# nianticlabs/implicit-depth

Hardware: AMD Instinct MI355X
Metric: frames/sec (BDModel.forward hot path, 512x384, 64 planes, 8-frame tuple = 1 current + 7 source views; third-party backbones excluded) (higher is better)
Workload: dtype f32

## Files before the change

implicit-depth_amd/csrc/conv.hip:

```cpp
#include <algorithm>
#include "conv_args.h"
#include "../../include/idh_ops.h"

using namespace idh_conv;

int idh_stem_op(const idh_op &op, hipStream_t st, bool launch);

namespace {

__device__ float g_zero_page[kZeroFloats];

thread_local bool t_dry_run = false;
thread_local int t_launches = 0;
#undef IDH_CHECK_LAUNCH
#define IDH_CHECK_LAUNCH()                                              \
    do {                                                                \
        if (!t_dry_run && hipGetLastError() != hipSuccess) return IDH_ELAUNCH; \
    } while (0)
#define IDH_LAUNCH(...)                         \
    do {                                        \
        if (t_dry_run) ++t_launches;            \
        else hipLaunchKernelGGL(__VA_ARGS__);   \
    } while (0)

// ... 1034 lines not shown
                ss[u][0] = fmaf(d0, d0, ss[u][0]); ss[u][1] = fmaf(d1, d1, ss[u][1]); ss[u][2] = fmaf(d2, d2, ss[u][2]); ss[u][3] = fmaf(d3, d3, ss[u][3]);
            }
        }
    }
#pragma unroll
    for (int u = 0; u < SUB; ++u) {
        float *mine = red + ((size_t)(prow + u * pstep) * cq + q) * 8;
#pragma unroll
        for (int e = 0; e < 4; ++e) { mine[e] = s[u][e]; mine[4 + e] = ss[u][e]; }
    }
    __syncthreads();
    for (int t = threadIdx.x; t < 8 * cq; t += blockDim.x) {
        const int qq = t >> 3, e = t & 7;
        float a = 0.f;
        for (int r = 0; r < rows; ++r) a += red[(r * cq + qq) * 8 + e];
        part[((size_t)(n * nchunks + chunk) * 2 + (e >> 2)) * C + 4 * qq + (e & 3)] = a;
    }
}

__global__ __launch_bounds__(256) void instnorm_finalize_k(const float *__restrict__ part, const float *__restrict__ in, int cs, int C, int HW,
                                                           int nchunks, float *__restrict__ stats) {
    const int n = blockIdx.x;
    for (int c = threadIdx.x; c < C; c += 256) {
        float s = 0.f, ss = 0.f;
        for (int k = 0; k < nchunks; ++k) {
            const float *o = part + ((size_t)(n * nchunks + k) * 2) * C + c;
            s += o[0];
            ss += o[C];
        }
        const float ms = s / (float)HW;
        const float var = fmaxf(ss / (float)HW - ms * ms, 0.f);
        stats[(size_t)n * 2 * C + c] = in[(size_t)n * HW * cs + c] + ms;
        stats[(size_t)n * 2 * C + C + c] = 1.0f / sqrtf(var + 1e-5f);
    }
}

__global__ __launch_bounds__(256) void instnorm_apply_k(const float *__restrict__ in, int cs, float *__restrict__ out, int out_cs,
                                                        int C, int HW, long long total, const float *__restrict__ stats, int act,
                                                        float slope) {
    const int cq = C >> 2;
    for (long long t = blockIdx.x * 256ll + threadIdx.x; t < total; t += gridDim.x * 256ll) {
        const int q = (int)(t % cq);
        const long long np = t / cq;
        const int n = (int)(np / HW);
        const float4 mean = *reinterpret_cast<const float4 *>(stats + (size_t)n * 2 * C + 4 * q);
        const float4 rstd = *reinterpret_cast<const float4 *>(stats + (size_t)n * 2 * C + C + 4 * q);
        const float4 v = *reinterpret_cast<const float4 *>(in + (size_t)np * cs + 4 * q);
        float r[4] = {(v.x - mean.x) * rstd.x, (v.y - mean.y) * rstd.y, (v.z - mean.z) * rstd.z, (v.w - mean.w) * rstd.w};
        for (int e = 0; e < 4; ++e) r[e] = act_apply(r[e], act, slope);
        *reinterpret_cast<float4 *>(out + (size_t)np * out_cs + 4 * q) = make_float4(r[0], r[1], r[2], r[3]);
    }
}

enum { LV_LDS4 = 0, LV_LDS2 = 1, LV_MFMA14 = 2, LV_UP2 = 3 };
struct LevelArgs {
    int n;
    unsigned start[kMaxGroup + 1];
    int kind[kMaxGroup];
    LdsConvArgs op[kMaxGroup];
};

template <bool WIDE>
__global__ __launch_bounds__(256) void level_k(const LevelArgs g) {
    __shared__ f32x4 sA[lds_a_slots(1)];
    __shared__ f32x4 sB[lds_b_slots(WIDE ? 4 : 2)];
    int idx = 0;
// ... 241 lines not shown
        g.start[i] = cursor;
        g.kind[i] = kinds[i];
        g.op[i] = pcs[i].la;
        if (kinds[i] == LV_MFMA14) g.op[i].c = pcs[i].a;
        cursor += pcs[i].blocks;
    }
    g.start[n] = cursor;
    bool wide = false;
    for (int i = 0; i < n; ++i) wide = wide || kinds[i] == LV_LDS4;
    if (wide) IDH_LAUNCH(level_k<true>, dim3(cursor), dim3(256), 0, st, g);
    else IDH_LAUNCH(level_k<false>, dim3(cursor), dim3(256), 0, st, g);
    IDH_CHECK_LAUNCH();
    return launch_reduces(pcs, n, st);
}

int level_kind(const PreparedConv &pc) {
    if (pc.up || pc.norm || pc.s2) return -1;
    if (pc.lds_rows == 4 && pc.nj == 4) return LV_LDS4;
    if (pc.lds_rows == 4 && pc.nj == 2) return LV_LDS2;
    if (pc.lds_rows == 0 && pc.tm == 1 && pc.tn == 4) return LV_MFMA14;
    return -1;
}

int check_upsample(const idh_op &op) {
    const idh_conv_src &s = op.src[0];
    if (!s.in || !op.out || (s.Cin & 3) || (s.cs & 3) || (op.out_cs & 3) || op.N <= 0 || s.H <= 0 || s.W <= 0 || s.Cin <= 0) return IDH_EINVAL;
    if ((long long)op.N * s.H * s.W * (s.Cin >> 2) >= (1ll << 31)) return IDH_EUNSUPPORTED;
    return IDH_OK;
}

constexpr unsigned kLevelMaxBlocks = 512;
constexpr unsigned kLevelUpsampleBlocks = 512;
constexpr long long kLevelUpsampleNatural = 4096;

}

extern "C" size_t idh_sizeof_op(void) { return sizeof(idh_op); }

extern "C" size_t idh_packed_weight_floats(int Cout, int Cin, int ks) {
    if (Cout <= 0 || Cin <= 0 || ks <= 0) return 0;
    return (size_t)ks * ks * ceil16(Cin) * ceil16(Cout);
}

extern "C" int idh_pack_conv_weight(const float *w, float *dst, int Cout, int Cin, int ks, void *stream) {
    if (!w || !dst || Cout <= 0 || Cin <= 0 || (ks != 1 && ks != 3)) return IDH_EINVAL;
    const long long total = (long long)idh_packed_weight_floats(Cout, Cin, ks);
    int grid = idh_cdiv(total, 256);
    if (grid > 4096) grid = 4096;
    hipLaunchKernelGGL(pack_weight_k, dim3(grid), dim3(256), 0, idh_stream(stream), w, dst, Cout, Cin, ks, ceil16(Cin),
                       ceil16(Cout));
    IDH_CHECK_LAUNCH();
    return IDH_OK;
}

extern "C" int idh_run_ops(const idh_op *ops, int n, void *stream) {
    if (n < 0 || (n > 0 && !ops)) return IDH_EINVAL;
    hipStream_t st = idh_stream(stream);
    for (int i = 0; i < n; ++i) {
        const idh_op &op = ops[i];
        const idh_conv_src &s = op.src[0];
        switch (op.kind) {
            case IDH_OP_CONV:
            case IDH_OP_UPSAMPLE2: {
                PreparedConv pcs[kMaxGroup];
                int kinds[kMaxGroup];
                int run = 0;
// ... 122 lines not shown
                IDH_CHECK_LAUNCH();
                break;
            }
            case IDH_OP_NHWC_TO_NCHW: {
                if (!s.in || !op.out || op.N <= 0 || op.N > 65535 || s.H <= 0 || s.W <= 0 || s.Cin <= 0 || s.cs < s.Cin) return IDH_EINVAL;
                const int HW = s.H * s.W;
                IDH_LAUNCH(export_nchw_k, dim3(idh_cdiv(HW, 64), idh_cdiv(s.Cin, 32), op.N), dim3(256), 0, st, s.in,
                                   op.out, s.Cin, HW, s.cs);
                IDH_CHECK_LAUNCH();
                break;
            }
            case IDH_OP_POINTWISE_HEAD: {
                if (!s.in || !s.w || !op.out || (s.Cin & 3) || (s.cs & 3) || op.N <= 0 || s.H <= 0 || s.W <= 0 || s.Cin <= 0 || s.cs < s.Cin)
                    return IDH_EINVAL;
                const long long M = (long long)op.N * s.H * s.W;
                int grid = idh_cdiv(M, 256);
                if (grid > 8192) grid = 8192;
                IDH_LAUNCH(pointwise_head_k, dim3(grid), dim3(256), 0, st, s.in, s.w, op.bias, op.out, op.ws, M, s.Cin,
                                   s.cs);
                IDH_CHECK_LAUNCH();
                break;
            }
            case IDH_OP_POINTWISE_NCHW: {
                if (!s.in || !s.w || !op.out || op.N <= 0 || s.H <= 0 || s.W <= 0 || (op.out_cs & 3) || ((uintptr_t)op.out & 15) ||
                    (op.bias && ((uintptr_t)op.bias & 15)))
                    return IDH_EINVAL;
                if (s.Cin != kPwCin || op.Cout != kPwCout || op.out_cs < kPwCout || (long long)s.H * s.W * kPwCin * 4 >= (1ll << 31))
                    return IDH_EUNSUPPORTED;
                PwNchwArgs pa{};
                pa.in = s.in; pa.w = s.w; pa.bias = op.bias; pa.out = op.out;
                pa.HW = s.H * s.W; pa.out_cs = op.out_cs;
                pa.tiles_per_img = idh_cdiv(pa.HW, kPwTile);
                pa.tiles = (long long)op.N * pa.tiles_per_img;
                const int grid = (int)std::min<long long>(pa.tiles, 256 * 4 * 4);
                IDH_LAUNCH(pointwise_nchw_k, dim3(grid), dim3(256), 0, st, pa);
                IDH_CHECK_LAUNCH();
                break;
            }
            case IDH_OP_POINTWISE_UP: {
                const idh_conv_src &lo = op.src[1];
                if (!s.in || !s.w || !lo.in || !op.out || op.N <= 0 || s.H <= 0 || s.W <= 0 || (s.H & 1) || (s.W & 1) || (s.cs & 3) || (lo.cs & 3) || (op.out_cs & 3) ||
                    s.cs < s.Cin || lo.cs < op.Cout || op.out_cs < op.Cout || ((uintptr_t)s.in & 15) || ((uintptr_t)lo.in & 15) || ((uintptr_t)op.out & 15) ||
                    ((uintptr_t)s.w & 15) || (op.bias && ((uintptr_t)op.bias & 15)) || lo.H != s.H / 2 || lo.W != s.W / 2)
                    return IDH_EINVAL;
                if (s.Cin != op.Cout || (s.Cin != 64 && s.Cin != 128) || (long long)s.H * s.W >= (1ll << 31)) return IDH_EUNSUPPORTED;
                PwUpArgs pa{};
                pa.in = s.in; pa.w = s.w; pa.bias = op.bias; pa.low = lo.in; pa.out = op.out;
                pa.H = s.H; pa.W = s.W; pa.in_cs = s.cs; pa.low_cs = lo.cs; pa.out_cs = op.out_cs;
                pa.tiles_per_img = idh_cdiv(s.H * s.W, kPwTile);
                pa.tiles = (long long)op.N * pa.tiles_per_img;
                const int grid = (int)std::min<long long>(pa.tiles, 256 * 8);
                if (s.Cin == 64) IDH_LAUNCH((pointwise_up_k<4, 4>), dim3(grid), dim3(256), 16 * 64 * sizeof(f32x4), st, pa);
                else IDH_LAUNCH((pointwise_up_k<8, 8>), dim3(grid), dim3(256), 32 * 128 * sizeof(f32x4), st, pa);
                IDH_CHECK_LAUNCH();
                break;
            }
            case IDH_OP_STEM: {
                const int rc = idh_stem_op(op, st, !t_dry_run);
                if (rc != IDH_OK) return rc;
                if (t_dry_run) ++t_launches;
                break;
            }
            case IDH_OP_COPY: {
                if (!s.in || !op.out || (s.Cin & 3) || (s.cs & 3) || (op.out_cs & 3) || op.N <= 0 || s.H <= 0 || s.W <= 0 || s.Cin <= 0 ||
                    s.cs < s.Cin || op.out_cs < s.Cin)
                    return IDH_EINVAL;
                const long long npix = (long long)op.N * s.H * s.W;
                int grid = idh_cdiv(npix * (s.Cin >> 2), 256);
                if (grid > 8192) grid = 8192;
                IDH_LAUNCH(copy_nhwc_k, dim3(grid), dim3(256), 0, st, s.in, op.out, npix, s.Cin, s.cs, op.out_cs);
                IDH_CHECK_LAUNCH();
                break;
            }
            case IDH_OP_INSTNORM: {
                const int C = s.Cin, HW = s.H * s.W;
                if (!s.in || !op.ws || C <= 0 || (C & 3) || 256 % (C >> 2) || (s.cs & 3) || (op.out && (op.out_cs & 3)) ||
                    op.N <= 0 || op.N > 65535 || s.H <= 0 || s.W <= 0)
                    return IDH_EINVAL;
                const int nchunks = idh_cdiv(HW, kInChunk);
                const int sthreads = ((long long)nchunks * op.N < 512 && C >= 64) ? 1024 : 256;
                if (C >= 64 && sthreads == 256)
                    IDH_LAUNCH(instnorm_stats_k<4>, dim3(nchunks, op.N), dim3(256), 1024 * 8 * sizeof(float), st, s.in, s.cs, C, HW, nchunks, op.ws);
                else
                    IDH_LAUNCH(instnorm_stats_k<1>, dim3(nchunks, op.N), dim3(sthreads), sthreads * 8 * sizeof(float), st, s.in, s.cs, C, HW,
                                       nchunks, op.ws);
                IDH_CHECK_LAUNCH();
                float *stats = op.ws + (size_t)op.N * nchunks * 2 * C;
                IDH_LAUNCH(instnorm_finalize_k, dim3(op.N), dim3(256), 0, st, op.ws, s.in, s.cs, C, HW, nchunks, stats);
                IDH_CHECK_LAUNCH();
                if (!op.out) break;
                const long long total = (long long)op.N * HW * (C >> 2);
                int gx = idh_cdiv(total, 256 * 4);
                if (gx > 16384) gx = 16384;
                IDH_LAUNCH(instnorm_apply_k, dim3(gx), dim3(256), 0, st, s.in, s.cs, op.out, op.out_cs, C, HW, total, stats, op.act,
                                   op.slope);
                IDH_CHECK_LAUNCH();
                break;
            }
            default:
                return IDH_EINVAL;
        }
    }
    return IDH_OK;
}

extern "C" int idh_conv_variant(const idh_op *op, int32_t out[8]) {
    if (!op || !out || op->kind != IDH_OP_CONV) return IDH_EINVAL;
    PreparedConv pc{};
    const int rc = prep_conv(*op, pc);
    if (rc != IDH_OK) return rc;
    const bool lds = pc.lds_rows == 8 || pc.lds_rows == 4;
    out[0] = pc.lds_rows;
    out[1] = lds ? pc.nj : 0;
    out[2] = lds ? 0 : pc.tm;
// ... 16 lines not shown
```

implicit-depth_amd/csrc/networks.hip:

```cpp
#include <algorithm>
#include <cstring>
#include <map>
#include <tuple>
#include <vector>

#include "idh_common.h"
#include "net_plan.h"
#include "../../include/idh_net.h"
#include "../../include/idh_ops.h"

namespace {

constexpr long long kReuseMinBytes = 64ll << 20;
constexpr bool kFuseHeadNorm = true;
constexpr bool kFuseHeadImport = true;

inline int ceil16(int v) { return (v + 15) & ~15; }
inline int cdiv(int a, int b) { return (a + b - 1) / b; }
inline size_t align64(size_t v) { return (v + 63) & ~(size_t)63; }

__global__ __launch_bounds__(256) void bias_sum_k(const float *__restrict__ a, const float *__restrict__ b, float *__restrict__ out, int n) {
    const int i = blockIdx.x * 256 + threadIdx.x;
    if (i < n) out[i] = (a ? a[i] : 0.f) + (b ? b[i] : 0.f);
}

enum Mode { MODE_SIZES, MODE_PACK, MODE_RUN };

struct Buf {
    float *base;
    int N, H, W, cs;
    bool internal;
    bool zero_fill;
    size_t floats;
};

struct View {
    int buf = -1, c0 = 0, C = 0;
};

struct Region {
    uint64_t buf, c0, c1;
};

struct Meta {
    std::vector<Region> reads, writes;
};

struct Src {
// ... 194 lines not shown
    }
    void export_nchw(const View &x, float *dst) {
        if (err) return;
        idh_op op;
        std::memset(&op, 0, sizeof op);
        op.kind = IDH_OP_NHWC_TO_NCHW; op.N = N(x);
        idh_conv_src &s = op.src[0];
        s.in = ptr(x); s.cs = cs(x); s.H = H(x); s.W = W(x); s.Cin = x.C;
        op.out = mode_ == MODE_RUN ? dst : reinterpret_cast<float *>(uintptr_t(4) << 32);
        ops.push_back(op);
        meta.push_back(Meta{{region(x)}, {}});
    }
    void head(const View &x, const idh_conv_params &cv, float *out, float *out_exp) {
        if (err) return;
        if (cv.cout != 1 || cv.ks != 1 || cv.cin != x.C) { err = IDH_EINVAL; return; }
        float *w = blob_alloc(cv.cin), *b = blob_alloc(1);
        if (mode_ == MODE_PACK) {
            if (!cv.weight || !cv.bias) { err = IDH_EINVAL; return; }
            if (hipMemcpyAsync(w, cv.weight, sizeof(float) * cv.cin, hipMemcpyDeviceToDevice, st_) != hipSuccess ||
                hipMemcpyAsync(b, cv.bias, sizeof(float), hipMemcpyDeviceToDevice, st_) != hipSuccess) err = IDH_ELAUNCH;
        }
        idh_op op;
        std::memset(&op, 0, sizeof op);
        op.kind = IDH_OP_POINTWISE_HEAD; op.N = N(x);
        idh_conv_src &s = op.src[0];
        s.in = ptr(x); s.w = w; s.cs = cs(x); s.H = H(x); s.W = W(x); s.Cin = x.C;
        op.bias = b;
        op.out = mode_ == MODE_RUN ? out : reinterpret_cast<float *>(uintptr_t(5) << 32);
        op.ws = mode_ == MODE_RUN ? out_exp : nullptr;
        ops.push_back(op);
        meta.push_back(Meta{{region(x)}, {}});
    }

    Norm instance_norm(const View &x, const View *out, int act, float slope) {
        Norm nm;
        if (err) return nm;
        if (x.C % 4 || 256 % (x.C / 4)) { err = IDH_EINVAL; return nm; }
        const int nchunks = cdiv(H(x) * W(x), 1024);
        float *w = ws_alloc((size_t)N(x) * (nchunks + 1) * 2 * x.C);
        idh_op op;
        std::memset(&op, 0, sizeof op);
        op.kind = IDH_OP_INSTNORM; op.N = N(x);
        idh_conv_src &s = op.src[0];
        s.in = ptr(x); s.cs = cs(x); s.H = H(x); s.W = W(x); s.Cin = x.C;
        op.act = act; op.slope = slope;
        if (out) { op.out = ptr(*out); op.out_cs = cs(*out); }
        op.ws = w;
        ops.push_back(op);
        Meta m{{region(x)}, {}};
        if (out) {
            m.writes.push_back(region(*out));
        } else {
            Buf b{};
            b.base = w + (size_t)N(x) * nchunks * 2 * x.C; b.N = N(x); b.H = 1; b.W = 1; b.cs = 1; b.internal = false;
            bufs.push_back(b);
            nm.stats = b.base; nm.buf = (int)bufs.size() - 1;
            m.writes.push_back(Region{(uint64_t)nm.buf, 0, 1});
        }
        meta.push_back(m);
        return nm;
    }
    static bool pointwise_nchw_eligible(const idh_conv_params &c) { return c.ks == 1 && c.stride == 1 && c.cin == 64 && c.cout == 128; }
    void pointwise_nchw(const float *src, int n, int C, int H_, int W_, const idh_conv_params &cv, const View &out) {
        if (err) return;
        if (n != N(out) || H_ != H(out) || W_ != W(out) || C != cv.cin || out.C != cv.cout || !pointwise_nchw_eligible(cv)) { err = IDH_EINVAL; return; }
        idh_op op;
        std::memset(&op, 0, sizeof op);
        op.kind = IDH_OP_POINTWISE_NCHW; op.N = n;
        idh_conv_src &s = op.src[0];
        s.in = mode_ == MODE_RUN ? src : reinterpret_cast<const float *>(uintptr_t(6) << 32);
        s.w = packed(cv, IDH_W_DIRECT); s.H = H_; s.W = W_; s.Cin = C; s.ks = 1; s.stride = 1;
        op.bias = bias_of(cv, nullptr);
        op.out = ptr(out); op.out_cs = cs(out); op.Ho = H_; op.Wo = W_; op.Cout = cv.cout;
        ops.push_back(op);
        meta.push_back(Meta{{}, {region(out)}});
    }

    void stem(const float *images, int n, int h, int w, const float *blob, const View &out) {
        if (err) return;
        idh_op op;
// ... 285 lines not shown
        if (i && (feats[i].H * 2 != feats[i - 1].H || feats[i].W * 2 != feats[i - 1].W)) return IDH_EINVAL;
        prev.push_back(input_view(p, feats[i], N));
    }
    return unetpp_body(p, blocks, heads, N, prev, fouts, log_depth, depth, nullptr, scales, true);
}

uint64_t layout_hash(const std::vector<idh_op> &ops) {
    uint64_t h = 1469598103934665603ull;
    auto mix = [&](long long v) {
        for (int i = 0; i < 8; ++i) { h ^= (uint64_t)((v >> (8 * i)) & 0xff); h *= 1099511628211ull; }
    };
    for (const idh_op &op : ops) {
        mix(op.kind); mix(op.N); mix(op.Ho); mix(op.Wo); mix(op.Cout); mix(op.tile_m); mix(op.tile_n); mix(op.split_k); mix(op.act); mix(op.group);
        for (const idh_conv_src &s : op.src) { mix(s.Cin); mix(s.H); mix(s.W); mix(s.cs); mix(s.ks); mix(s.stride); mix(s.pad_mode); mix(s.norm != nullptr); }
    }
    return h;
}

}

int idh_internal::conv_stage(int mode, ConvStage *s, float *ws, size_t ws_cap, float *blob, hipStream_t st, int (*before_ops)(void *), void *ctx) {
    const Mode m = mode == STAGE_SIZES ? MODE_SIZES : mode == STAGE_PACK ? MODE_PACK : MODE_RUN;
    if (!s || !s->enc || s->n_enc != 4 || !s->dec || s->N <= 0 || s->H <= 0 || s->W <= 0 || s->D <= 0) return IDH_EINVAL;
    Plan p(m, ws, ws_cap, blob, st);
    s->match = nullptr;
    s->n_head_ops = 0;
    if (s->head_mode) {
        if (!s->head || s->K <= 0 || (s->head_mode != 1 && s->head_mode != 2)) return IDH_EINVAL;
        const idh_conv_params &c1 = s->head[0], &c2 = s->head[1];
        const int M = s->N * (s->K + 1), H = s->H, W = s->W;
        if (c1.ks != 1 || c1.stride != 1 || c2.ks != 3 || c2.stride != 1 || c2.cin != c1.cout) return IDH_EINVAL;
        if (m == MODE_RUN && (!s->layer1 || ((uintptr_t)s->layer1 & 15))) return IDH_EINVAL;
        const View h = p.buffer(M, H, W, c1.cout);
        if (s->head_mode == 1 && kFuseHeadImport && Plan::pointwise_nchw_eligible(c1)) {
            p.pointwise_nchw(s->layer1, M, c1.cin, H, W, c1, h);
        } else {
            View x;
            if (s->head_mode == 1) {
                x = p.buffer(M, H, W, c1.cin);
                p.import_nchw(s->layer1, M, c1.cin, H, W, x);
            } else {
                const idh_tensor t{const_cast<float *>(s->layer1), IDH_LAYOUT_NHWC, c1.cin, H, W, c1.cin};
                if (!tensor_ok(&t, m == MODE_RUN)) return IDH_EINVAL;
                x = p.external(t, M);
            }
            p.conv(x, c1, h, IDH_ACT_NONE, 0.2f, nullptr, nullptr, nullptr);
        }
        const View y = p.buffer(M, H, W, c2.cout);
        idh_conv_choice hc;
        if (p.select({{h, &c2}}, y, IDH_ACT_NONE, 0.2f, nullptr, IDH_PAD_REPLICATE, false, false, &hc) != IDH_OK) return IDH_EINVAL;
        if (kFuseHeadNorm && h.C % 16 == 0 && hc.lds_subtiles == 1 && (hc.families & IDH_FAMILY_LDS)) {
            const Norm nm = p.instance_norm(h, nullptr, IDH_ACT_NONE, 0.2f);
            Norm on = nm;
            on.act = IDH_ACT_LRELU; on.slope = 0.2f;
            p.conv(h, c2, y, IDH_ACT_NONE, 0.2f, nullptr, nullptr, nullptr, IDH_PAD_REPLICATE, &on);
        } else {
            const View hn = p.buffer(M, H, W, c1.cout);
            p.instance_norm(h, &hn, IDH_ACT_LRELU, 0.2f);
            p.conv(hn, c2, y, IDH_ACT_NONE, 0.2f, nullptr, nullptr, nullptr, IDH_PAD_REPLICATE);
        }
        const View mo = p.buffer(M, H, W, c2.cout);
        p.instance_norm(y, &mo, IDH_ACT_NONE, 0.2f);
        if (p.err) return p.err;
        if (p.cs(mo) != mo.C) return IDH_EUNSUPPORTED;
        s->match = p.ptr(mo);
        s->n_head_ops = (int)p.ops.size();
    }
    const View cv_in = p.buffer(s->N, s->H, s->W, s->D);
    for (int i = 0; i < 5; ++i)
        if (s->img[i].layout != IDH_LAYOUT_NCHW || !tensor_ok(&s->img[i], m == MODE_RUN)) return IDH_EINVAL;
    const View v0 = input_view(p, s->img[0], s->N);
    std::vector<View> levels{v0};
    int rc = cvencoder_body(p, s->enc, s->n_enc, s->N, cv_in, &s->img[1], nullptr, &levels);
    if (rc != IDH_OK) return rc;
    for (int i = 1; i < 5; ++i)
        if (p.H(levels[i]) * 2 != p.H(levels[i - 1]) || p.W(levels[i]) * 2 != p.W(levels[i - 1])) return IDH_EINVAL;
    View f0;
    rc = unetpp_body(p, s->dec, s->heads, s->N, levels, nullptr, s->log_depth, s->depth, &f0, s->scales);
    if (rc != IDH_OK) return rc;
    s->cv_in = p.ptr(cv_in);
    s->cv_cs = p.cs(cv_in);
    s->feat0 = p.ptr(f0);
    s->feat0_cs = p.cs(f0); s->feat0_C = f0.C; s->feat0_H = p.H(f0); s->feat0_W = p.W(f0);
    for (int i = 0; i < 5; ++i) { s->level_H[i] = p.H(levels[i]); s->level_W[i] = p.W(levels[i]); }
    p.before_run = before_ops;
    p.before_ctx = ctx;
    idh_net_sizes sz{};
    if (m == MODE_PACK) return p.err;
    rc = p.finish(m == MODE_SIZES ? &sz : nullptr, s->n_head_ops);
    if (rc != IDH_OK) return rc;
    if (m == MODE_SIZES) {
// ... 116 lines not shown
```

implicit-depth_amd/nhwc.py:

```python
from __future__ import annotations

import ctypes as C
from dataclasses import dataclass
from typing import Dict, List, Optional, Sequence

import torch
from torch import nn

from . import _lib

OP_CONV, OP_UPSAMPLE2, OP_IMPORT, OP_EXPORT, OP_SPLITK, OP_HEAD, OP_INSTNORM, OP_UPSAMPLE2_NEAREST, OP_COPY, OP_POINTWISE_NCHW, OP_POINTWISE_UP = 1, 2, 3, 4, 5, 6, 7, 8, 9, 10, 11
OP_STEM = 12
ACT_NONE, ACT_LRELU, ACT_ELU = 0, 1, 2
PAD_ZEROS, PAD_REPLICATE = 0, 1


class ConvSrc(C.Structure):
    _fields_ = [("in_", C.c_void_p), ("w", C.c_void_p), ("cs", C.c_int32), ("H", C.c_int32), ("W", C.c_int32),
                ("Cin", C.c_int32), ("ks", C.c_int32), ("stride", C.c_int32), ("pad_mode", C.c_int32), ("_r", C.c_int32),
                ("up_in", C.c_void_p * 2), ("up_cs", C.c_int32 * 2), ("up_c0", C.c_int32), ("up_C", C.c_int32),
                ("norm", C.c_void_p), ("norm_slope", C.c_float), ("norm_act", C.c_int32)]


class Op(C.Structure):
    _fields_ = [("kind", C.c_int32), ("N", C.c_int32), ("src", ConvSrc * 2), ("bias", C.c_void_p), ("res", C.c_void_p),
                ("out", C.c_void_p), ("ws", C.c_void_p), ("res_cs", C.c_int32), ("out_cs", C.c_int32), ("Ho", C.c_int32),
                ("Wo", C.c_int32), ("Cout", C.c_int32), ("act", C.c_int32), ("slope", C.c_float), ("split_k", C.c_int32),
                ("tile_m", C.c_int32), ("tile_n", C.c_int32), ("group", C.c_int32)]


def _bind():
    return _lib.lib()


@dataclass
class View:

    buf: torch.Tensor
    c0: int
    C: int

    @property
    def N(self):
        return self.buf.shape[0]

# ... 151 lines not shown
            raise _lib.IdhError("the fused second source of a split-precision conv must be a 1x1 conv with the same Cout")
        ci1 = w1.shape[1]
        w1c = w1.detach().reshape(co, ci1).contiguous()
    n = L.idh_packed_split_weight_bytes(co, ci, ci1, SPLIT_CODE[math])
    if kh != 3 or kw != 3 or n == 0:
        raise _lib.IdhError("split-precision conv covers 3x3 kernels with Cout % 64 == 0")
    dst = torch.empty(n // 4, device=w.device, dtype=torch.int32)
    wc = w.detach().contiguous()
    _lib.check(L.idh_pack_conv_weight_split(wc.data_ptr(), _lib.ptr(w1c), dst.data_ptr(), co, ci, ci1, SPLIT_CODE[math], _lib.stream_ptr()),
               "idh_pack_conv_weight_split")
    conv._idh_packed_split = (key, dst)
    return dst


MATH_MODES = ("fp32", "f16x3")
DEFAULT_MATH = "fp32"
SPLIT_MIN_BLOCKS = 256


def split_eligible(srcs, cout: int, N: int, Ho: int, Wo: int, pad_mode: int) -> bool:
    return bool(select(srcs, cout, N, Ho, Wo, pad_mode).families & FAMILY_SPLIT)


def choose_split_rows(N: int, Ho: int, Wo: int, cout: int) -> int:
    return select([(None, _conv_shape(16, 3))], cout, N, Ho, Wo).split_rows


FUSE_UPSAMPLE = False
FUSED_UP_ROWS = 4

MERGE_LEVELS = True
FUSE_HEAD_NORM = True
FUSE_HEAD_IMPORT = True

TARGET_WAVES = 2048
MIN_WAVES = 1024


def lds_eligible(srcs, cout: int, Wo: int, pad_mode: int) -> bool:
    return bool(select(srcs, cout, 1, 1, Wo, pad_mode).families & FAMILY_LDS)


S2_FIRST = True
S2_FIRST_MIN_BLOCKS = 512


def s2_first_eligible(srcs, cout: int, N: int, Ho: int, Wo: int, pad_mode: int) -> bool:
    return bool(select(srcs, cout, N, Ho, Wo, pad_mode).families & FAMILY_S2_FIRST)


def lds_subtiles(cout: int) -> int:
    return select([(None, _conv_shape(16, 3))], cout, 1, 1, 1).lds_subtiles


NARROW_TILE_BELOW = 400
NARROWEST_TILE_BELOW = 0


SPLIT_MIN_CHUNKS = 6
SPLIT_MAX = 16
PROJ_LOWRES = False
PROJ_LOWRES_MIN_TILES = 1536
PROJ_CHUNK_WEIGHT = 0.5


def choose_lds_tile(N: int, Ho: int, Wo: int, cout: int, chunks: int):
# ... 146 lines not shown
    def upsample2(self, x: View, out: View, nearest: bool = False):
        op = Op()
        op.kind, op.N = (OP_UPSAMPLE2_NEAREST if nearest else OP_UPSAMPLE2), x.N
        s = op.src[0]
        s.in_, s.cs, s.H, s.W, s.Cin = x.ptr, x.cs, x.H, x.W, x.C
        op.out, op.out_cs = out.ptr, out.cs
        self.ops.append(op)
        self.meta.append({"reads": [_region(x)], "writes": [_region(out)]})
        self._arr = None
        return out

    def pointwise_up(self, x: View, conv: nn.Conv2d, low: View, out: View):
        if conv.kernel_size[0] != 1 or conv.in_channels != x.C or conv.out_channels != out.C or low.C != out.C or (2 * low.H, 2 * low.W) != (x.H, x.W):
            raise _lib.IdhError("pointwise_up: a 1x1 conv of x plus the x2 upsampling of a half-resolution map with the output's channels")
        op = Op()
        op.kind, op.N = OP_POINTWISE_UP, x.N
        w = packed_weight(conv)
        self.keep.append(w)
        s = op.src[0]
        s.in_, s.w, s.cs, s.H, s.W, s.Cin, s.ks, s.stride = x.ptr, w.data_ptr(), x.cs, x.H, x.W, x.C, 1, 1
        l = op.src[1]
        l.in_, l.cs, l.H, l.W, l.Cin = low.ptr, low.cs, low.H, low.W, low.C
        if conv.bias is not None:
            b = conv.bias.detach().contiguous()
            self.keep.append(b)
            op.bias = b.data_ptr()
        op.out, op.out_cs, op.Ho, op.Wo, op.Cout = out.ptr, out.cs, out.H, out.W, out.C
        self.flops += 2 * x.N * x.H * x.W * conv.out_channels * conv.in_channels
        self.ops.append(op)
        self.meta.append({"reads": [_region(x), _region(low)], "writes": [_region(out)]})
        self._arr = None
        return out

    def instance_norm(self, x: View, out: Optional[View], act=ACT_NONE, slope=0.2):
        if x.C % 4 or 256 % (x.C // 4):
            raise _lib.IdhError(f"instance-norm kernel needs C/4 to divide 256 (C={x.C})")
        op = Op()
        op.kind, op.N = OP_INSTNORM, x.N
        s = op.src[0]
        s.in_, s.cs, s.H, s.W, s.Cin = x.ptr, x.cs, x.H, x.W, x.C
        op.act, op.slope = act, slope
        if out is not None:
            op.out, op.out_cs = out.ptr, out.cs
        nchunks = -(-(x.H * x.W) // 1024)
        ws = torch.empty(x.N * (nchunks + 1) * 2 * x.C, device=self.device, dtype=torch.float32)
        self.keep.append(ws)
        op.ws = ws.data_ptr()
        self.ops.append(op)
        stats = ws[x.N * nchunks * 2 * x.C:].view(x.N, 2, x.C)
        self.meta.append({"reads": [_region(x)], "writes": [_region(out)] if out is not None else [(stats.data_ptr(), 0, 1)]})
        self._arr = None
        return out if out is not None else stats

    def copy(self, x: View, out: View):
        if (x.N, x.H, x.W, x.C) != (out.N, out.H, out.W, out.C):
            raise _lib.IdhError("copy: shape mismatch")
        op = Op()
        op.kind, op.N = OP_COPY, x.N
        s = op.src[0]
        s.in_, s.cs, s.H, s.W, s.Cin = x.ptr, x.cs, x.H, x.W, x.C
        op.out, op.out_cs = out.ptr, out.cs
        self.ops.append(op)
        self.meta.append({"reads": [_region(x)], "writes": [_region(out)]})
        self._arr = None
        return out

    def import_nchw(self, shape_nchw, out: View) -> int:
        N, Cc, H, W = [int(v) for v in shape_nchw]
        if (N, H, W, Cc) != (out.N, out.H, out.W, out.C):
            raise _lib.IdhError(f"import of {tuple(shape_nchw)} into a view of {(out.N, out.C, out.H, out.W)}")
        op = Op()
        op.kind, op.N = OP_IMPORT, N
        s = op.src[0]
        s.H, s.W, s.Cin = H, W, Cc
        op.out, op.out_cs = out.ptr, out.cs
        self.ops.append(op)
        self.meta.append({"reads": [], "writes": [_region(out)]})
        self._arr = None
        return len(self.ops) - 1

# ... 220 lines not shown
        self.d = collections.OrderedDict()

    def get(self, key):
        ent = self.d.get(key)
        if ent is not None:
            self.d.move_to_end(key)
        return ent

    @staticmethod
    def _same_shapes(a, b) -> bool:
        return (isinstance(a, tuple) and isinstance(b, tuple) and len(a) == len(b) and
                all(x == y or (isinstance(x, ParamKey) and isinstance(y, ParamKey)) for x, y in zip(a, b)))

    def put(self, key, ent):
        for k in [k for k in self.d if k != key and self._same_shapes(k, key)]:
            del self.d[k]
        self.d[key] = ent
        self.d.move_to_end(key)
        while len(self.d) > self.entries:
            self.d.popitem(last=False)
        return ent

    def values(self):
        return self.d.values()

    def __len__(self):
        return len(self.d)

    def clear(self):
        self.d.clear()


def build_flags() -> tuple:
    return (WINO_GROUP, FUSE_UPSAMPLE, FUSED_UP_ROWS, MERGE_LEVELS, FUSE_HEAD_NORM, FUSE_HEAD_IMPORT, NARROW_TILE_BELOW, NARROWEST_TILE_BELOW, SPLIT_MIN_CHUNKS,
            SPLIT_MAX, SPLIT_MIN_BLOCKS, WINOGRAD, WINO_MIN_TILES, WINO_MIN_FILL, WINOGRAD4, WINOGRAD4_PROJ, WINO4_MIN_TILES, WINO4_MIN_FILL, BUFFER_REUSE, REUSE_MIN_BYTES, DEFAULT_MATH,
            S2_FIRST, S2_FIRST_MIN_BLOCKS, PROJ_CHUNK_WEIGHT, PROJ_LOWRES, PROJ_LOWRES_MIN_TILES)


def _plan_cache(module: nn.Module) -> PlanCache:
    c = module.__dict__.get("_idh_plans")
    if c is None:
        c = PlanCache()
        module.__dict__["_idh_plans"] = c
        _lib.watch_state_dict_loads(module)
    return c


def _param_key(module: nn.Module):
    return ParamKey((math_of(module), build_flags()) + tuple((p.data_ptr(), _lib.param_version(p)) for p in module.parameters()))


def _check_in(*ts):
    for t in ts:
        _lib.require_cuda_f32(t)
        if t.dim() != 4:
            raise _lib.IdhError(f"expected NCHW tensors, got shape {tuple(t.shape)}")


def block_forward_nchw(blk, x: torch.Tensor) -> torch.Tensor:
    _check_in(x)
    x = x.contiguous()
    key = ("bb", tuple(x.shape), str(x.device), _param_key(blk))
    cache = _plan_cache(blk)
    ent = cache.get(key)
    if ent is None:
        p = Plan(x.device, math=math_of(blk))
        N, Cc, H, W = x.shape
# ... 146 lines not shown
            if getattr(dec, "depth_head", False):
                i_out[i] = p.head(v, dec.convs[f"output_{i}"][1], torch.empty(1, device=feats[0].device))
            else:
                i_out[i] = p.export_nchw(v)
        p.schedule()
        ent = (p, i_in, i_out, final)
        cache.put(key, ent)
    p, i_in, i_out, final = ent
    for i, f in zip(i_in, feats):
        p.set_in(i, f)
    res = {}
    for i, v in final.items():
        ch = 1 if getattr(dec, "depth_head", False) else v.C
        t = torch.empty(v.N, ch, v.H, v.W, device=feats[0].device, dtype=torch.float32)
        p.set_out(i_out[i], t)
        res[dec.out_key.format(i)] = t
    p.run()
    return res


def binary_mlp_forward(net, inputs, max_scale_only):
    from .mlp import binary_mlp_forward as f

    return f(net, inputs, max_scale_only)


def norm_on_load_eligible(p: Plan, x: View, conv: nn.Conv2d, pad_mode: int) -> bool:
    return (p.math == "fp32" and x.C % 16 == 0 and lds_subtiles(conv.out_channels) == 1 and
            lds_eligible([(x, conv)], conv.out_channels, x.W, pad_mode))


def build_matching_head(p: Plan, enc, x: Optional[View], nchw_shape=None):
    c1, c2 = enc.net[5], enc.net[8]
    if nchw_shape is not None:
        N, _, H, W = [int(v) for v in nchw_shape]
        h = p.buffer(N, H, W, c1.out_channels)
        i_in = p.pointwise_nchw(nchw_shape, c1, h)
        x = h
    else:
        h = p.buffer(x.N, x.H, x.W, c1.out_channels)
        p.conv(x, c1, h)
    y = p.buffer(x.N, x.H, x.W, c2.out_channels)
    if FUSE_HEAD_NORM and norm_on_load_eligible(p, h, c2, PAD_REPLICATE):
        stats = p.instance_norm(h, None)
        p.conv(h, c2, y, pad_mode=PAD_REPLICATE, norm=(stats, ACT_LRELU, 0.2))
    else:
        hn = p.buffer(x.N, x.H, x.W, c1.out_channels)
        p.instance_norm(h, hn, act=ACT_LRELU, slope=0.2)
        p.conv(hn, c2, y, pad_mode=PAD_REPLICATE)
    out = p.buffer(x.N, x.H, x.W, c2.out_channels)
    p.instance_norm(y, out)
    return out if nchw_shape is None else (out, i_in)


def matching_head_forward(enc, feat_nchw: torch.Tensor, channels_last: bool = False) -> torch.Tensor:
    _check_in(feat_nchw)
    x = feat_nchw.contiguous()
    key = ("mh", tuple(x.shape), str(x.device), channels_last, _param_key(enc.net[5]) + _param_key(enc.net[8]))
    cache = _plan_cache(enc)
    ent = cache.get(key)
    if ent is None:
        p = Plan(x.device, math=math_of(enc))
        N, Cc, H, W = x.shape
        if FUSE_HEAD_IMPORT and Plan.pointwise_nchw_eligible(enc.net[5]):
            y, i_in = build_matching_head(p, enc, None, nchw_shape=x.shape)
        else:
            xin = p.buffer(N, H, W, Cc)
            i_in = p.import_nchw(x.shape, xin)
            y = build_matching_head(p, enc, xin)
        i_out = None if channels_last else p.export_nchw(y)
        p.schedule()
        ent = (p, i_in, i_out, y)
        cache.put(key, ent)
    p, i_in, i_out, y = ent
    p.set_in(i_in, x)
    if channels_last:
        p.run()
        return y.dense().clone()
    out = torch.empty(y.N, y.C, y.H, y.W, device=x.device, dtype=torch.float32)
    p.set_out(i_out, out)
    p.run()
# ... 208 lines not shown
```

include/idh_ops.h:

```cpp
#ifndef IDH_OPS_H_
#define IDH_OPS_H_

#include <stddef.h>
#include <stdint.h>

#ifdef __cplusplus
extern "C" {
#endif
#if defined(__GNUC__) || defined(__clang__)
#pragma GCC visibility push(default)
#endif

enum {
    IDH_OP_CONV = 1,
    IDH_OP_UPSAMPLE2 = 2,
    IDH_OP_NCHW_TO_NHWC = 3,
    IDH_OP_NHWC_TO_NCHW = 4,
    IDH_OP_SPLITK_REDUCE = 5,
    IDH_OP_POINTWISE_HEAD = 6,
    IDH_OP_COPY = 9,
    IDH_OP_UPSAMPLE2_NEAREST = 8,
    IDH_OP_POINTWISE_NCHW = 10,
    IDH_OP_POINTWISE_UP = 11,
    IDH_OP_STEM = 12,
    IDH_OP_INSTNORM = 7
};

#define IDH_PAD_ZEROS 0
#define IDH_PAD_REPLICATE 1

typedef struct idh_conv_src {
    const float *in;
    const float *w;
    int32_t cs, H, W, Cin;
    int32_t ks, stride, pad_mode, _r;
    const float *up_in[2];
    int32_t up_cs[2];
    int32_t up_c0, up_C;
    const float *norm;
    float norm_slope;
    int32_t norm_act;
} idh_conv_src;

typedef struct idh_op {
    int32_t kind;
    int32_t N;
    idh_conv_src src[2];
    const float *bias;
    const float *res;
    float *out;
    float *ws;
    int32_t res_cs, out_cs;
    int32_t Ho, Wo, Cout;
    int32_t act;
    float slope;
    int32_t split_k;
    int32_t tile_m, tile_n;
    int32_t group;
} idh_op;
// ... 88 lines not shown
```

Before: 688.7.

## Fuse instance-norm partial statistics into the matching-head pointwise NCHW conv

Adds a pointwise NCHW conv kernel that also accumulates per-chunk shifted sum and sum-of-squares partials while writing its output. The following instance-norm op then skips its separate stats pass and goes straight to finalize. This removes one full read of the 128-channel head activation and one kernel launch. In exchange the grid is fixed to one block per chunk per image instead of a capped persistent grid, and the kernel carries the extra reduction work and register pressure.

```diff
diff --git a/implicit-depth_amd/csrc/conv.hip b/implicit-depth_amd/csrc/conv.hip
--- a/implicit-depth_amd/csrc/conv.hip
+++ b/implicit-depth_amd/csrc/conv.hip
@@ -1090,6 +1090,109 @@
         const float var = fmaxf(ss / (float)HW - ms * ms, 0.f);
         stats[(size_t)n * 2 * C + c] = in[(size_t)n * HW * cs + c] + ms;
         stats[(size_t)n * 2 * C + C + c] = 1.0f / sqrtf(var + 1e-5f);
+    }
+}
+
+struct PwNchwStatsArgs {
+    const float *in, *w, *bias;
+    float *out, *part;
+    int HW, out_cs, nchunks;
+};
+
+__global__ __launch_bounds__(256, 4) void pointwise_nchw_stats_k(const PwNchwStatsArgs a) {
+    constexpr int C16 = kPwCin / 16, NT = kPwCout / 32, kRows = 32;
+    static_assert(kRows * kPwCout * 2 * sizeof(float) <= (kPwCin / 4) * kPwCout * sizeof(f32x4), "the row partials reuse the weights' LDS");
+    __shared__ f32x4 sW[(kPwCin / 4) * kPwCout];
+    {
+        const f32x4 *g = reinterpret_cast<const f32x4 *>(a.w);
+        for (int i = threadIdx.x; i < (kPwCin / 4) * kPwCout; i += 256) sW[i] = g[i];
+    }
+    __syncthreads();
+    const int lane = threadIdx.x & 63;
+    const int wave = __builtin_amdgcn_readfirstlane(threadIdx.x >> 6);
+    const int ln = lane & 15, h = lane >> 4;
+    const int n = blockIdx.y, chunk = blockIdx.x;
+    const int p0 = chunk * kInChunk, p1 = min(a.HW, p0 + kInChunk);
+    const int prow = 16 * (wave & 1) + ln;
+    const int cb = 64 * (wave >> 1);
+
+    const unsigned img_bytes = (unsigned)kPwCin * (unsigned)a.HW * 4u;
+    const __amdgpu_buffer_rsrc_t rs = __builtin_amdgcn_make_buffer_rsrc(const_cast<float *>(a.in + (size_t)n * kPwCin * a.HW), 0, img_bytes, 0x00020000);
+    auto load = [&](int p, f32x4 (&x)[C16]) {
+        const int voff = p < a.HW ? (4 * h * a.HW + p) * 4 : (int)0x7fffffff;
+#pragma unroll
+        for (int c = 0; c < C16; ++c)
+#pragma unroll
+            for (int e = 0; e < 4; ++e)
+                x[c][e] = __builtin_bit_cast(float, __builtin_amdgcn_raw_buffer_load_b32(rs, voff, (16 * c + e) * a.HW * 4, 0));
+    };
+    auto conv = [&](const f32x4 (&x)[C16], f32x4 (&v)[NT]) {
+#pragma unroll
+        for (int j = 0; j < NT; ++j) v[j] = (f32x4){0.f, 0.f, 0.f, 0.f};
+        int opaque = 0;
+        asm volatile("" : "+s"(opaque));
+        const f32x4 *sWt = sW + opaque;
+#pragma unroll
+        for (int c = 0; c < C16; ++c)
+#pragma unroll
+            for (int j = 0; j < NT; ++j) {
+                const f32x4 A = sWt[(4 * c + h) * kPwCout + cb + 16 * j + ln];
+#pragma unroll
+                for (int kk = 0; kk < 4; ++kk) v[j] = __builtin_amdgcn_mfma_f32_16x16x4f32(A[kk], x[c][kk], v[j], 0, 0, 0);
+            }
+        if (a.bias) {
+#pragma unroll
+            for (int j = 0; j < NT; ++j) v[j] += *reinterpret_cast<const f32x4 *>(a.bias + cb + 16 * j + 4 * h);
+        }
+    };
+
+    f32x4 xa[C16], xb[C16], piv[NT], s[NT], ss[NT];
+    load(0, xa);
+    conv(xa, piv);
+#pragma unroll
+    for (int j = 0; j < NT; ++j) s[j] = ss[j] = (f32x4){0.f, 0.f, 0.f, 0.f};
+    auto tile = [&](int p, const f32x4 (&x)[C16]) {
+        f32x4 v[NT];
+        conv(x, v);
+        if (p < p1) {
+            float *o = a.out + ((size_t)n * a.HW + p) * a.out_cs + cb + 4 * h;
+#pragma unroll
+            for (int j = 0; j < NT; ++j) {
+                *reinterpret_cast<f32x4 *>(o + 16 * j) = v[j];
+#pragma unroll
+                for (int e = 0; e < 4; ++e) {
+                    const float d = v[j][e] - piv[j][e];
+                    s[j][e] += d;
+                    ss[j][e] = fmaf(d, d, ss[j][e]);
+                }
+            }
+        }
+    };
+    const int ntiles = (p1 - p0 + kRows - 1) / kRows;
+    load(p0 + prow, xa);
+    for (int t = 0;; t += 2) {
+        const int p = p0 + kRows * t + prow;
+        if (t + 1 < ntiles) load(p + kRows, xb);
+        tile(p, xa);
+        if (t + 1 >= ntiles) break;
+        if (t + 2 < ntiles) load(p + 2 * kRows, xa);
+        tile(p + kRows, xb);
+        if (t + 2 >= ntiles) break;
+    }
+
+    __syncthreads();
+    float *red = reinterpret_cast<float *>(sW);
+#pragma unroll
+    for (int j = 0; j < NT; ++j) {
+        *reinterpret_cast<f32x4 *>(red + prow * kPwCout + cb + 16 * j + 4 * h) = s[j];
+        *reinterpret_cast<f32x4 *>(red + (kRows + prow) * kPwCout + cb + 16 * j + 4 * h) = ss[j];
+    }
+    __syncthreads();
+    {
+        const int c = threadIdx.x & (kPwCout - 1), e = threadIdx.x >> 7;
+        float acc = 0.f;
+        for (int r = 0; r < kRows; ++r) acc += red[(e * kRows + r) * kPwCout + c];
+        a.part[((size_t)(n * a.nchunks + chunk) * 2 + e) * kPwCout + c] = acc;
     }
 }
 
@@ -1397,6 +1500,12 @@
 constexpr unsigned kLevelMaxBlocks = 512;
 constexpr unsigned kLevelUpsampleBlocks = 512;
 constexpr long long kLevelUpsampleNatural = 4096;
+
+bool head_partials_pair(const idh_op &pw, const idh_op &nm) {
+    const idh_conv_src &ps = pw.src[0], &ns = nm.src[0];
+    return pw.ws && nm.ws == pw.ws && nm.tile_m == IDH_NORM_PARTIALS && pw.N == nm.N && pw.N <= 65535 && ns.Cin == kPwCout && pw.Cout == kPwCout &&
+           (long long)ps.H * ps.W == (long long)ns.H * ns.W && ns.in == pw.out && ns.cs == pw.out_cs;
+}
 
 }
 
@@ -1585,6 +1694,18 @@
                 pa.HW = s.H * s.W; pa.out_cs = op.out_cs;
                 pa.tiles_per_img = idh_cdiv(pa.HW, kPwTile);
                 pa.tiles = (long long)op.N * pa.tiles_per_img;
+                if (op.ws) {
+                    const idh_op *nm = nullptr;
+                    for (int j = i + 1; j < n && !nm; ++j)
+                        if (ops[j].kind == IDH_OP_INSTNORM && ops[j].ws == op.ws) nm = &ops[j];
+                    if (!nm || !head_partials_pair(op, *nm)) return IDH_EINVAL;
+                    PwNchwStatsArgs sa{};
+                    sa.in = s.in; sa.w = s.w; sa.bias = op.bias; sa.out = op.out; sa.part = op.ws;
+                    sa.HW = pa.HW; sa.out_cs = op.out_cs; sa.nchunks = idh_cdiv(pa.HW, kInChunk);
+                    IDH_LAUNCH(pointwise_nchw_stats_k, dim3(sa.nchunks, op.N), dim3(256), 0, st, sa);
+                    IDH_CHECK_LAUNCH();
+                    break;
+                }
                 const int grid = (int)std::min<long long>(pa.tiles, 256 * 4 * 4);
                 IDH_LAUNCH(pointwise_nchw_k, dim3(grid), dim3(256), 0, st, pa);
                 IDH_CHECK_LAUNCH();
@@ -1632,7 +1753,12 @@
                     return IDH_EINVAL;
                 const int nchunks = idh_cdiv(HW, kInChunk);
                 const int sthreads = ((long long)nchunks * op.N < 512 && C >= 64) ? 1024 : 256;
-                if (C >= 64 && sthreads == 256)
+                if (op.tile_m == IDH_NORM_PARTIALS) {
+                    const idh_op *pw = nullptr;
+                    for (int j = i - 1; j >= 0 && !pw; --j)
+                        if (ops[j].kind == IDH_OP_POINTWISE_NCHW && ops[j].ws == op.ws) pw = &ops[j];
+                    if (!pw || !head_partials_pair(*pw, op)) return IDH_EINVAL;
+                } else if (C >= 64 && sthreads == 256)
                     IDH_LAUNCH(instnorm_stats_k<4>, dim3(nchunks, op.N), dim3(256), 1024 * 8 * sizeof(float), st, s.in, s.cs, C, HW, nchunks, op.ws);
                 else
                     IDH_LAUNCH(instnorm_stats_k<1>, dim3(nchunks, op.N), dim3(sthreads), sthreads * 8 * sizeof(float), st, s.in, s.cs, C, HW,
diff --git a/implicit-depth_amd/csrc/networks.hip b/implicit-depth_amd/csrc/networks.hip
--- a/implicit-depth_amd/csrc/networks.hip
+++ b/implicit-depth_amd/csrc/networks.hip
@@ -14,6 +14,7 @@
 constexpr long long kReuseMinBytes = 64ll << 20;
 constexpr bool kFuseHeadNorm = true;
 constexpr bool kFuseHeadImport = true;
+constexpr bool kFuseHeadStats = true;
 
 inline int ceil16(int v) { return (v + 15) & ~15; }
 inline int cdiv(int a, int b) { return (a + b - 1) / b; }
@@ -274,7 +275,7 @@
         meta.push_back(Meta{{region(x)}, {}});
     }
 
-    Norm instance_norm(const View &x, const View *out, int act, float slope) {
+    Norm instance_norm(const View &x, const View *out, int act, float slope, int producer = -1) {
         Norm nm;
         if (err) return nm;
         if (x.C % 4 || 256 % (x.C / 4)) { err = IDH_EINVAL; return nm; }
@@ -288,6 +289,12 @@
         op.act = act; op.slope = slope;
         if (out) { op.out = ptr(*out); op.out_cs = cs(*out); }
         op.ws = w;
+        if (producer >= 0) {
+            idh_op &pw = ops[(size_t)producer];
+            if (pw.kind != IDH_OP_POINTWISE_NCHW || pw.out != ptr(x) || pw.out_cs != cs(x) || pw.N != N(x) || x.C != 128) { err = IDH_EINVAL; return nm; }
+            pw.ws = w;
+            op.tile_m = IDH_NORM_PARTIALS;
+        }
         ops.push_back(op);
         Meta m{{region(x)}, {}};
         if (out) {
@@ -639,8 +646,10 @@
         if (c1.ks != 1 || c1.stride != 1 || c2.ks != 3 || c2.stride != 1 || c2.cin != c1.cout) return IDH_EINVAL;
         if (m == MODE_RUN && (!s->layer1 || ((uintptr_t)s->layer1 & 15))) return IDH_EINVAL;
         const View h = p.buffer(M, H, W, c1.cout);
+        int prod = -1;
         if (s->head_mode == 1 && kFuseHeadImport && Plan::pointwise_nchw_eligible(c1)) {
             p.pointwise_nchw(s->layer1, M, c1.cin, H, W, c1, h);
+            if (kFuseHeadStats && !p.err) prod = (int)p.ops.size() - 1;
         } else {
             View x;
             if (s->head_mode == 1) {
@@ -657,13 +666,13 @@
         idh_conv_choice hc;
         if (p.select({{h, &c2}}, y, IDH_ACT_NONE, 0.2f, nullptr, IDH_PAD_REPLICATE, false, false, &hc) != IDH_OK) return IDH_EINVAL;
         if (kFuseHeadNorm && h.C % 16 == 0 && hc.lds_subtiles == 1 && (hc.families & IDH_FAMILY_LDS)) {
-            const Norm nm = p.instance_norm(h, nullptr, IDH_ACT_NONE, 0.2f);
+            const Norm nm = p.instance_norm(h, nullptr, IDH_ACT_NONE, 0.2f, prod);
             Norm on = nm;
             on.act = IDH_ACT_LRELU; on.slope = 0.2f;
             p.conv(h, c2, y, IDH_ACT_NONE, 0.2f, nullptr, nullptr, nullptr, IDH_PAD_REPLICATE, &on);
         } else {
             const View hn = p.buffer(M, H, W, c1.cout);
-            p.instance_norm(h, &hn, IDH_ACT_LRELU, 0.2f);
+            p.instance_norm(h, &hn, IDH_ACT_LRELU, 0.2f, prod);
             p.conv(hn, c2, y, IDH_ACT_NONE, 0.2f, nullptr, nullptr, nullptr, IDH_PAD_REPLICATE);
         }
         const View mo = p.buffer(M, H, W, c2.cout);
diff --git a/implicit-depth_amd/nhwc.py b/implicit-depth_amd/nhwc.py
--- a/implicit-depth_amd/nhwc.py
+++ b/implicit-depth_amd/nhwc.py
@@ -11,6 +11,7 @@
 
 OP_CONV, OP_UPSAMPLE2, OP_IMPORT, OP_EXPORT, OP_SPLITK, OP_HEAD, OP_INSTNORM, OP_UPSAMPLE2_NEAREST, OP_COPY, OP_POINTWISE_NCHW, OP_POINTWISE_UP = 1, 2, 3, 4, 5, 6, 7, 8, 9, 10, 11
 OP_STEM = 12
+NORM_PARTIALS = 1
 ACT_NONE, ACT_LRELU, ACT_ELU = 0, 1, 2
 PAD_ZEROS, PAD_REPLICATE = 0, 1
 
@@ -228,6 +229,7 @@
 MERGE_LEVELS = True
 FUSE_HEAD_NORM = True
 FUSE_HEAD_IMPORT = True
+FUSE_HEAD_STATS = True
 
 TARGET_WAVES = 2048
 MIN_WAVES = 1024
@@ -440,7 +442,7 @@
         self._arr = None
         return out
 
-    def instance_norm(self, x: View, out: Optional[View], act=ACT_NONE, slope=0.2):
+    def instance_norm(self, x: View, out: Optional[View], act=ACT_NONE, slope=0.2, producer: Optional[int] = None):
         if x.C % 4 or 256 % (x.C // 4):
             raise _lib.IdhError(f"instance-norm kernel needs C/4 to divide 256 (C={x.C})")
         op = Op()
@@ -454,6 +456,11 @@
         ws = torch.empty(x.N * (nchunks + 1) * 2 * x.C, device=self.device, dtype=torch.float32)
         self.keep.append(ws)
         op.ws = ws.data_ptr()
+        if producer is not None:
+            pw = self.ops[producer]
+            if pw.kind != OP_POINTWISE_NCHW or pw.out != x.ptr or pw.out_cs != x.cs or pw.N != x.N or x.C != 128:
+                raise _lib.IdhError("instance_norm: producer must be the pointwise_nchw op that writes this 128-channel view")
+            pw.ws, op.tile_m = op.ws, NORM_PARTIALS
         self.ops.append(op)
         stats = ws[x.N * nchunks * 2 * x.C:].view(x.N, 2, x.C)
         self.meta.append({"reads": [_region(x)], "writes": [_region(out)] if out is not None else [(stats.data_ptr(), 0, 1)]})
@@ -740,7 +747,7 @@
 
 
 def build_flags() -> tuple:
-    return (WINO_GROUP, FUSE_UPSAMPLE, FUSED_UP_ROWS, MERGE_LEVELS, FUSE_HEAD_NORM, FUSE_HEAD_IMPORT, NARROW_TILE_BELOW, NARROWEST_TILE_BELOW, SPLIT_MIN_CHUNKS,
+    return (WINO_GROUP, FUSE_UPSAMPLE, FUSED_UP_ROWS, MERGE_LEVELS, FUSE_HEAD_NORM, FUSE_HEAD_IMPORT, FUSE_HEAD_STATS, NARROW_TILE_BELOW, NARROWEST_TILE_BELOW, SPLIT_MIN_CHUNKS,
             SPLIT_MAX, SPLIT_MIN_BLOCKS, WINOGRAD, WINO_MIN_TILES, WINO_MIN_FILL, WINOGRAD4, WINOGRAD4_PROJ, WINO4_MIN_TILES, WINO4_MIN_FILL, BUFFER_REUSE, REUSE_MIN_BYTES, DEFAULT_MATH,
             S2_FIRST, S2_FIRST_MIN_BLOCKS, PROJ_CHUNK_WEIGHT, PROJ_LOWRES, PROJ_LOWRES_MIN_TILES)
 
@@ -953,21 +960,23 @@
 
 def build_matching_head(p: Plan, enc, x: Optional[View], nchw_shape=None):
     c1, c2 = enc.net[5], enc.net[8]
+    prod = None
     if nchw_shape is not None:
         N, _, H, W = [int(v) for v in nchw_shape]
         h = p.buffer(N, H, W, c1.out_channels)
         i_in = p.pointwise_nchw(nchw_shape, c1, h)
+        prod = i_in if FUSE_HEAD_STATS else None
         x = h
     else:
         h = p.buffer(x.N, x.H, x.W, c1.out_channels)
         p.conv(x, c1, h)
     y = p.buffer(x.N, x.H, x.W, c2.out_channels)
     if FUSE_HEAD_NORM and norm_on_load_eligible(p, h, c2, PAD_REPLICATE):
-        stats = p.instance_norm(h, None)
+        stats = p.instance_norm(h, None, producer=prod)
         p.conv(h, c2, y, pad_mode=PAD_REPLICATE, norm=(stats, ACT_LRELU, 0.2))
     else:
         hn = p.buffer(x.N, x.H, x.W, c1.out_channels)
-        p.instance_norm(h, hn, act=ACT_LRELU, slope=0.2)
+        p.instance_norm(h, hn, act=ACT_LRELU, slope=0.2, producer=prod)
         p.conv(hn, c2, y, pad_mode=PAD_REPLICATE)
     out = p.buffer(x.N, x.H, x.W, c2.out_channels)
     p.instance_norm(y, out)
diff --git a/include/idh_ops.h b/include/idh_ops.h
--- a/include/idh_ops.h
+++ b/include/idh_ops.h
@@ -25,6 +25,7 @@
     IDH_OP_STEM = 12,
     IDH_OP_INSTNORM = 7
 };
+#define IDH_NORM_PARTIALS 1
 
 #define IDH_PAD_ZEROS 0
 #define IDH_PAD_REPLICATE 1
```

Result: no change. 693.8 (median of 6 runs) (+0.7%).
